# PRBonn/SHINE_mapping

Hardware: NVIDIA H100
Metric: sdf_train_points_per_sec_fwd_bwd (higher is better)
Workload: dtype f32

## Files before the change

### include/shine_b200.h

```cpp
#ifndef SHINE_B200_H_
#define SHINE_B200_H_

#include <stdint.h>

#ifdef __cplusplus
extern "C" {
#endif

#define SHINE_ABI_VERSION 5
#define SHINE_MAX_LEVELS 8
#define SHINE_HASH_SLOT_BYTES 64

#define SHINE_OK 0
#define SHINE_ERR_INVALID_ARG (-1)
#define SHINE_ERR_UNSUPPORTED (-2)
#define SHINE_ERR_CAPACITY (-3)

#define SHINE_FLAG_REDUCTION_SUM 1u
#define SHINE_FLAG_WEIGHTED 2u
#define SHINE_FLAG_TF32X1 4u
#define SHINE_FLAG_MORTON_ORDERED 16u
#define SHINE_FLAG_LOSS_L2 32u
#define SHINE_FLAG_LOSS_L1 64u

// ... 18 lines not shown

typedef struct shine_decoder {
    const float *w1, *b1, *w2, *b2, *w3, *b3;
    float *gw1, *gb1, *gw2, *gb2, *gw3, *gb3;
    int32_t in_dim;
    int32_t hidden;
    int32_t mlp_level;
    int32_t reserved;
} shine_decoder;

int shine_abi_version(void);
const char* shine_error_string(int code);

int shine_hash_insert(void* slots, uint32_t capacity, const int64_t* keys, const int32_t* corner_ids,
                      int64_t n, int32_t node_base, int32_t* overflow_count, void* stream);

int shine_points_to_morton(const float* coord, int64_t n, int32_t level, int64_t* morton, void* stream);

int shine_get_indices(const shine_octree* oct, const float* coord, int64_t n, int64_t* out_idx, void* stream);

int shine_query_fwd(const shine_octree* oct, const float* coord, int64_t n, float* out_feat, void* stream);

int shine_query_bwd(const shine_octree* oct, const float* coord, int64_t n, const float* dfeat, void* stream);

int shine_query_coord_grad(const shine_octree* oct, const float* coord, int64_t n, const float* dfeat,
                           float* out_dcoord, void* stream);
int shine_query_tangent_fwd(const shine_octree* oct, const float* coord, int64_t n, const float* tangent,
                            float* out_feat, void* stream);
int shine_query_tangent_bwd(const shine_octree* oct, const float* coord, int64_t n, const float* tangent,
                            const float* dfeat, void* stream);

int shine_sdf_infer(const shine_octree* oct, const shine_decoder* dec, const float* coord, int64_t n,
                    float* out_pred, uint8_t* out_mask, int32_t mask_level, uint32_t flags, void* stream);

int shine_sdf_fwd(const shine_octree* oct, const shine_decoder* dec, const float* coord, const float* label,
                  const float* weight, int64_t n, float sigma, float scale, float loss_scale, float* out_pred,
                  float* out_loss, uint32_t flags, void* stream);

int shine_sdf_step(const shine_octree* oct, const shine_decoder* dec, const float* coord, const float* label,
                   const float* weight, int64_t n, float sigma, float scale, float loss_scale, const float* d_loss,
                   float* out_pred, float* out_loss, uint32_t flags, void* stream);

int shine_sdf_bce_fwd(const shine_octree* oct, const shine_decoder* dec, const float* coord,
                      const float* label, const float* weight, int64_t n, float sigma, float loss_scale,
                      float* out_pred, float* out_loss, uint32_t flags, void* stream);

int shine_reduce_grad_replicas(const shine_octree* oct, void* stream);

#define SHINE_ADAM_MAX_TENSORS 16
typedef struct shine_adam_tensor {
    float* param; float* grad; float* exp_avg; float* exp_avg_sq;
    int64_t numel; float lr; float weight_decay;
} shine_adam_tensor;
int shine_adam_step(const shine_adam_tensor* tensors, int32_t count, float beta1, float beta2, float eps,
                    int32_t step, int32_t zero_grad, void* stream);

int shine_adam_step_dev(const shine_adam_tensor* tensors, int32_t count, float beta1, float beta2, float eps,
                        void* state, int32_t zero_grad, void* stream);

typedef struct shine_build_level {
    void* node_slots;
    void* corner_slots;
    void* frame_node_set;
    void* frame_corner_set;
    int32_t* node_ids_out;
    int64_t* corner_morton_out;
// ... 214 lines not shown
```

### shine_mapping_b200/_abi.py

```python
from __future__ import annotations

import ctypes as C
import os

import torch

_HERE = os.path.dirname(os.path.abspath(__file__))
LIB_PATH = os.environ.get("SHINE_B200_LIB") or os.path.join(_HERE, "csrc", "libshine_b200.so")

ABI_VERSION = 5
MAX_LEVELS = 8
HASH_SLOT_BYTES = 64
ADAM_MAX_TENSORS = 16
FLAG_REDUCTION_SUM = 1
FLAG_WEIGHTED = 2
FLAG_TF32X1 = 4
FLAG_MORTON_ORDERED = 16
FLAG_LOSS_L2 = 32
FLAG_LOSS_L1 = 64
ERR_CAPACITY = -3
REGISTER_OUT = 29
REGISTER_SCRATCH_BYTES = 1024 * REGISTER_OUT * 8
RAYCAST_MAX_REFINE = 32
CAMERA_PINHOLE = 0
# ... 76 lines not shown
class ShineCamera(C.Structure):
    _fields_ = [("model", C.c_int32), ("width", C.c_int32), ("height", C.c_int32), ("fx", C.c_float), ("fy", C.c_float),
                ("cx", C.c_float), ("cy", C.c_float), ("fov_up", C.c_float), ("fov_down", C.c_float)]


class ShineHostPool(C.Structure):
    _fields_ = [("chunks", C.c_void_p), ("chunk_shift", C.c_int32), ("num_chunks", C.c_int32), ("size", C.c_int64)]


class ShineScanInput(C.Structure):
    _fields_ = [("records", C.c_void_p), ("n", C.c_int64), ("stride_bytes", C.c_int32), ("fp64", C.c_int32)]


class ShineBrickGrid(C.Structure):
    _fields_ = [("bricks", C.c_void_p), ("sdf", C.c_void_p), ("mask", C.c_void_p), ("all_keys", C.c_void_p),
                ("num_all", C.c_int64), ("num_bricks", C.c_int64), ("origin", C.c_float * 3), ("spacing", C.c_float),
                ("n", C.c_int32), ("lo", C.c_int32 * 3), ("hi", C.c_int32 * 3), ("missing_sdf", C.c_float)]


_vp, _i64, _i32, _u32, _f32 = C.c_void_p, C.c_int64, C.c_int32, C.c_uint32, C.c_float
_OCT, _DEC = C.POINTER(ShineOctree), C.POINTER(ShineDecoder)
SYMBOLS = {
    "shine_abi_version": (C.c_int, []),
    "shine_error_string": (C.c_char_p, [C.c_int]),
    "shine_hash_insert": (C.c_int, [_vp, _u32, _vp, _vp, _i64, _i32, _vp, _vp]),
    "shine_points_to_morton": (C.c_int, [_vp, _i64, _i32, _vp, _vp]),
    "shine_get_indices": (C.c_int, [_OCT, _vp, _i64, _vp, _vp]),
    "shine_query_fwd": (C.c_int, [_OCT, _vp, _i64, _vp, _vp]),
    "shine_query_bwd": (C.c_int, [_OCT, _vp, _i64, _vp, _vp]),
    "shine_query_coord_grad": (C.c_int, [_OCT, _vp, _i64, _vp, _vp, _vp]),
    "shine_query_tangent_fwd": (C.c_int, [_OCT, _vp, _i64, _vp, _vp, _vp]),
    "shine_query_tangent_bwd": (C.c_int, [_OCT, _vp, _i64, _vp, _vp, _vp]),
    "shine_sdf_infer": (C.c_int, [_OCT, _DEC, _vp, _i64, _vp, _vp, _i32, _u32, _vp]),
    "shine_sdf_fwd": (C.c_int, [_OCT, _DEC, _vp, _vp, _vp, _i64, _f32, _f32, _f32, _vp, _vp, _u32, _vp]),
    "shine_sdf_step": (C.c_int, [_OCT, _DEC, _vp, _vp, _vp, _i64, _f32, _f32, _f32, _vp, _vp, _vp, _u32, _vp]),
    "shine_sdf_bce_fwd": (C.c_int, [_OCT, _DEC, _vp, _vp, _vp, _i64, _f32, _f32, _vp, _vp, _u32, _vp]),
    "shine_reduce_grad_replicas": (C.c_int, [_OCT, _vp]),
    "shine_octree_frame_nodes": (C.c_int, [C.POINTER(ShineBuild), _vp, _i64, _vp]),
    "shine_octree_frame_corners": (C.c_int, [C.POINTER(ShineBuild), _i32, _vp]),
    "shine_octree_sort_scratch_bytes": (C.c_int64, [_i32]),
    "shine_octree_sort_new_keys": (C.c_int, [_vp, _vp, _i32, _vp, _i64, _vp]),
    "shine_octree_assign_rows": (C.c_int, [C.POINTER(ShineBuild), _vp, _i32, _vp]),
    "shine_octree_fill_nodes": (C.c_int, [C.POINTER(ShineBuild), _vp, _i32, _vp, _vp]),
    "shine_octree_corner_rehash": (C.c_int, [_vp, _u32, _vp, _i64, _vp]),
    "shine_count_positive": (C.c_int, [_vp, _i64, _vp, _vp]),
    "shine_sdf_eikonal_step": (C.c_int, [_OCT, _DEC, _vp, _vp, _vp, _i64, _f32, _f32, _f32, _f32, _vp, _vp, _vp, _vp, _vp,
                                         _u32, _vp]),
    "shine_mark_touched": (C.c_int, [_OCT, _vp, _i64, C.POINTER(ShineTouched), _vp]),
    "shine_regularization_apply": (C.c_int, [_OCT, C.POINTER(ShineTouched), C.POINTER(ShineRowTables), _f32, _vp, _i32, _vp]),
    "shine_importance_accumulate": (C.c_int, [_OCT, C.POINTER(ShineTouched), C.POINTER(ShineRowTables), _i32, _i32, _vp]),
    "shine_boundary_pack": (C.c_int, [C.POINTER(ShineBoundary), _i32, _i32, _vp, _vp]),
    "shine_boundary_unpack": (C.c_int, [C.POINTER(ShineBoundary), _i32, _i32, _vp, _vp]),
    "shine_nccl_unique_id": (C.c_int, [_vp]),
    "shine_nccl_comm_create": (C.c_int, [_vp, _i32, _i32, _i32, C.POINTER(C.c_void_p)]),
    "shine_nccl_comm_destroy": (C.c_int, [_vp]),
    "shine_allreduce_decoder_grads": (C.c_int, [_vp, _vp, _i64, _vp]),
    "shine_comm_last_error": (C.c_char_p, []),
    "shine_p2p_create": (C.c_int, [_i32, _i32, _i32, _i64, _vp, C.POINTER(C.c_void_p)]),
    "shine_p2p_connect": (C.c_int, [_vp, _vp]),
    "shine_p2p_exchange": (C.c_int, [_vp, _vp, _i64, C.POINTER(ShineBoundary), C.POINTER(ShineBoundaryInverse), _i32, _i32, _vp]),
    "shine_p2p_timeouts": (C.c_int, [_vp, C.POINTER(C.c_int32)]),
    "shine_p2p_destroy": (C.c_int, [_vp]),
    "shine_adam_step": (C.c_int, [C.POINTER(ShineAdamTensor), _i32, _f32, _f32, _f32, _i32, _i32, _vp]),
    "shine_adam_step_dev": (C.c_int, [C.POINTER(ShineAdamTensor), _i32, _f32, _f32, _f32, _vp, _i32, _vp]),
    "shine_pool_scratch_bytes": (C.c_int64, [_i64]),
    "shine_pool_window_append": (C.c_int, [C.POINTER(ShineSamplePool), _vp, _vp, _vp, _i64, _f32, _f32, _f32, _f32, _vp,
# ... 83 lines not shown
```

### shine_mapping_b200/csrc/shine_b200.cu

```cuda

#include <cuda_runtime.h>
#include <math.h>
#include <stdint.h>

#include <type_traits>

#include "shine_b200.h"

#ifndef SHINE_GATHER_GROUP
#define SHINE_GATHER_GROUP 2
#endif
#ifndef SHINE_TRAIN_MINB
#define SHINE_TRAIN_MINB 2
#endif
#ifndef SHINE_TRAIN_DECGRAD_MINB
#define SHINE_TRAIN_DECGRAD_MINB 1
#endif
#ifndef SHINE_INFER_MINB
#define SHINE_INFER_MINB 3
#endif

#include "shine_device.cuh"

namespace {
// ... 255 lines not shown
    const float2 v = *reinterpret_cast<const float2*>(blk + 2 * c);
    split_fast2(v.x, v.y, bh.x, bh.y, bl.x, bl.y);
}
__device__ __forceinline__ void stage_afrags(float* blk, const int (&sq)[2], const float (&c)[4][4]) {
#pragma unroll
    for (int mt = 0; mt < 2; ++mt)
#pragma unroll
        for (int q = 0; q < 2; ++q)
            *reinterpret_cast<float4*>(blk + 128 * mt + 4 * sq[q]) = make_float4(c[2 * mt][q], c[2 * mt + 1][q], c[2 * mt][2 + q], c[2 * mt + 1][2 + q]);
}
__device__ __forceinline__ int xfrag_word(int ks, int c) { return 64 * ks + 2 * (c ^ (8 * ks)); }
__device__ __forceinline__ void load_xfrag(const float* sx, int ks, int c, uint2& bh, uint2& bl) {
    const float2 v = *reinterpret_cast<const float2*>(sx + xfrag_word(ks, c));
    split_fast2(v.x, v.y, bh.x, bh.y, bl.x, bl.y);
}


constexpr int kGatherGroup = SHINE_GATHER_GROUP;

using shine_internal::StepParams;

struct SmemPlan {
    static constexpr int W1 = 0;
    static constexpr int W1T = W1 + 2 * kH * kF;
    static constexpr int W2 = W1T + 2 * kF * kWS;
    static constexpr int W3W2T = W2 + 2 * kH * kWS;
    static constexpr int B1 = W3W2T + 2 * kH * kWS;
    static constexpr int B2 = B1 + kH;
    static constexpr int W3 = B2 + kH;
    static constexpr int B3 = W3 + kH;
    static constexpr int GSCALE = B3 + 1;
    static constexpr int kDecGradFloats = kH * kF + kH + kH * kH + kH + kH + 1;
    static constexpr int ZSUM = B3 + 4;
    static constexpr int H1Z = ZSUM + 8;
    static constexpr int H2Z = H1Z + kH;
    static constexpr int D2Z = H2Z + kH;
    static constexpr int DB1Z = D2Z + kH;
    static constexpr int kZsumFloats = 8 * 5 * kTile;
    static_assert(DB1Z + kH <= ZSUM + kZsumFloats, "g0 fits the zero-tile corner");
    static constexpr int STAGE = ZSUM + kZsumFloats;
    static constexpr int SB2 = 0;
    static constexpr int SU = SB2;
    static constexpr int SA1 = SB2 + kTile * kH;
    static constexpr int SX = SA1 + kTile * kH;
    static constexpr int SA2 = SX + kTile * kF;
    static constexpr int SDP = SA2;
    static constexpr int kStagePerWarp = SA2 + kTile * kH;
    static constexpr int kStageGrouped = SDP + 2 * kTile;
    __host__ __device__ static constexpr int stage_per_warp(bool grouped) { return grouped ? kStageGrouped : kStagePerWarp; }
    static constexpr int kGroupPerLevel = 4 * kTile;
    static constexpr int kW2Part = kH * kH;
};

__device__ __forceinline__ void zero_tile_gradient(float* smem, const float* __restrict__ w2, int lane) {
    const float h1 = fmaxf(smem[SmemPlan::B1 + lane], 0.f);
    float a2 = smem[SmemPlan::B2 + lane];
#pragma unroll
    for (int k = 0; k < kH; ++k) a2 = fmaf(__ldg(w2 + lane * kH + k), __shfl_sync(kFull, h1, k), a2);
    const float d2 = a2 > 0.f ? smem[SmemPlan::W3 + lane] : 0.f;
    float db1 = 0.f;
#pragma unroll
    for (int n = 0; n < kH; ++n) db1 = fmaf(__ldg(w2 + n * kH + lane), __shfl_sync(kFull, d2, n), db1);
    smem[SmemPlan::H1Z + lane] = h1;
    smem[SmemPlan::H2Z + lane] = fmaxf(a2, 0.f);
    smem[SmemPlan::D2Z + lane] = d2;
    smem[SmemPlan::DB1Z + lane] = h1 > 0.f ? db1 : 0.f;
}
__device__ __forceinline__ float zero_tile_sum_and_gradient(float* smem, const float* __restrict__ w2, int warp, int lane) {
    float s = 0.f;
#pragma unroll
    for (int w = 0; w < 8; ++w) s += smem[SmemPlan::ZSUM + w];
    if (s != 0.f) {
        if (warp == 0) zero_tile_gradient(smem, w2, lane);
        __syncthreads();
    }
    return s;
}

constexpr int kMaxGroupedRuns = 6;

__device__ __forceinline__ void red_add_f2(float* p, float a, float b) {
    asm volatile("red.global.add.v2.f32 [%0], {%1,%2};" ::"l"(p), "f"(a), "f"(b) : "memory");
}
__device__ __forceinline__ int group_slot(int p) { return 4 * (p & 3) + (p >> 2); }

template <int LMAX>
__device__ __forceinline__ void grouped_scatter(const StepParams& P, int L, int tile, const float* __restrict__ pt,
                                                float* __restrict__ dtile, const float (&dxc)[4], int lane) {
    const int g = lane >> 2, t = lane & 3;
    *reinterpret_cast<float2*>(dtile + g * kF + 2 * t) = make_float2(dxc[0], dxc[1]);
    *reinterpret_cast<float2*>(dtile + (g + 8) * kF + 2 * t) = make_float2(dxc[2], dxc[3]);
    __syncwarp();
    uint2 bh[2], bl[2];
#pragma unroll
    for (int c = 0; c < 2; ++c)
        split_fast2(dtile[(8 * c + t) * kF + g], dtile[(8 * c + t + 4) * kF + g], bh[c].x, bh[c].y, bl[c].x, bl[c].y);
    const float sx = (g & 4) ? 1.f : -1.f, ox = (g & 4) ? 0.f : 1.f;
    const float sy = (g & 2) ? 1.f : -1.f, oy = (g & 2) ? 0.f : 1.f;
    const float sz = (g & 1) ? 1.f : -1.f, oz = (g & 1) ? 0.f : 1.f;
    const int id_off = 8 * (g & 1) + 4 + (g >> 1);
    const int own = group_slot(lane & 15);
#pragma unroll
    for (int i = 0; i < LMAX; ++i) {
        if (i >= L) break;
// ... 68 lines not shown
            if (v2 >= 0) {
                const int row = __ldg(slot_words + 16 * (int64_t)v2 + id_off);
                red_add_f2(gb + (int64_t)row * kF + 2 * t, c0[2] + c1[2], c0[3] + c1[3]);
            }
        }
    }
    __syncwarp();
}

struct BatchCoords {
    __device__ __forceinline__ void load(const StepParams& P, int64_t p, float& x, float& y, float& z) const {
        x = __ldg(P.coord + 3 * p); y = __ldg(P.coord + 3 * p + 1); z = __ldg(P.coord + 3 * p + 2);
    }
    __device__ __forceinline__ float out(float v) const { return v; }
};
struct GridCoords {
    shine_internal::BrickGrid g;
    __device__ __forceinline__ void load(const StepParams&, int64_t p, float& x, float& y, float& z) const {
        const int n1 = g.n + 1, per = n1 * n1 * n1;
        const int64_t b = p / per;
        const int r = (int)(p - b * per);
        const int i = r / (n1 * n1), j = (r / n1) % n1, k = r % n1;
        x = __fadd_rn(g.origin[0], __fmul_rn(g.spacing, (float)(__ldg(g.bricks + 3 * b) * g.n + i)));
        y = __fadd_rn(g.origin[1], __fmul_rn(g.spacing, (float)(__ldg(g.bricks + 3 * b + 1) * g.n + j)));
        z = __fadd_rn(g.origin[2], __fmul_rn(g.spacing, (float)(__ldg(g.bricks + 3 * b + 2) * g.n + k)));
    }
    __device__ __forceinline__ float out(float v) const { return -v; }
};

template <class Src>
constexpr int infer_min_blocks() { return std::is_same<Src, BatchCoords>::value ? SHINE_INFER_MINB : 2; }

template <int NTF, bool TRAIN, bool DEC_GRAD, int LMAX, bool GROUPED = false, class Src = BatchCoords, int LOSS = kLossBce>
__global__ void __launch_bounds__(256, !TRAIN ? infer_min_blocks<Src>() : (DEC_GRAD && !GROUPED) ? SHINE_TRAIN_DECGRAD_MINB : SHINE_TRAIN_MINB)
sdf_fused_kernel(const __grid_constant__ StepParams P, const __grid_constant__ Src src) {
    static_assert(std::is_same<Src, BatchCoords>::value || !TRAIN, "generated coordinates are for inference only");
    static_assert(!GROUPED || TRAIN, "the grouped scatter belongs to the training kernels");
    static_assert(!DEC_GRAD || TRAIN, "decoder gradients belong to the training kernels");
    static_assert(LOSS == kLossBce || std::is_same<Src, BatchCoords>::value, "the loss belongs to labelled batches");
    static_assert(SmemPlan::kStagePerWarp >= SmemPlan::kDecGradFloats, "a warp's staging area holds its partial decoder gradient");
    static_assert(SmemPlan::kStageGrouped >= kH * kF + 3 * kH + 1, "a grouped warp's staging area holds its partial bias / dW1 gradients");
    static_assert(!(GROUPED && DEC_GRAD) ||
                      (SmemPlan::STAGE + 8 * (SmemPlan::kStageGrouped + LMAX * SmemPlan::kGroupPerLevel + SmemPlan::kW2Part)) * 4 + 1024 <=
                          227 * 1024 / SHINE_TRAIN_MINB,
                  "the grouped kernel's shared memory fits SHINE_TRAIN_MINB blocks/SM");
    extern __shared__ __align__(16) float smem[];
    uint32_t* smu = reinterpret_cast<uint32_t*>(smem);
    const int tid = threadIdx.x, lane = tid & 31, warp = tid >> 5;
    const int g = lane >> 2, t = lane & 3, odd = t & 1, half = t >> 1;
    constexpr int kWarps = 8;

    for (int i = tid; i < kH * kF; i += blockDim.x) {
        const int nrow = i / kF, k = i % kF;
        uint32_t hi, lo; split_tf32(P.dec.w1[i], hi, lo);
        smu[SmemPlan::W1 + i] = hi; smu[SmemPlan::W1 + kH * kF + i] = lo;
        smu[SmemPlan::W1T + k * kWS + nrow] = hi; smu[SmemPlan::W1T + kF * kWS + k * kWS + nrow] = lo;
    }
    for (int i = tid; i < kH * kH; i += blockDim.x) {
        const int nrow = i / kH, k = i % kH;
        const float w = P.dec.w2[i];
        uint32_t hi, lo; split_tf32(w, hi, lo);
        smu[SmemPlan::W2 + nrow * kWS + k] = hi; smu[SmemPlan::W2 + kH * kWS + nrow * kWS + k] = lo;
        split_tf32(__fmul_rn(P.dec.w3[nrow], w), hi, lo);
        smu[SmemPlan::W3W2T + k * kWS + nrow] = hi; smu[SmemPlan::W3W2T + kH * kWS + k * kWS + nrow] = lo;
    }
    if (tid < kH) {
        smem[SmemPlan::B1 + tid] = P.dec.b1 ? P.dec.b1[tid] : 0.f;
        smem[SmemPlan::B2 + tid] = P.dec.b2 ? P.dec.b2[tid] : 0.f;
        smem[SmemPlan::W3 + tid] = P.dec.w3[tid];
    }
    if (tid == 0) {
        smem[SmemPlan::B3] = P.dec.b3 ? P.dec.b3[0] : 0.f;
        smem[SmemPlan::GSCALE] = P.loss_scale * ((TRAIN && P.d_loss) ? __ldg(P.d_loss) : 1.0f);
    }
    constexpr int kPark = LMAX <= 4 ? 16 : 32;
    constexpr int kIdPark = 4 * LMAX;
    __syncthreads();
    SHINE_ACC_DECL;
#pragma unroll
    for (int a = 0; a < 2; ++a) {
#pragma unroll
        for (int b = 0; b < 4; ++b) { dW2[a][b][0] = dW2[a][b][1] = dW2[a][b][2] = dW2[a][b][3] = 0.f; }
        dW1[a][0] = dW1[a][1] = dW1[a][2] = dW1[a][3] = 0.f;
    }
#pragma unroll
    for (int j = 0; j < 4; ++j) { db2p[j][0] = db2p[j][1] = db1p[j][0] = db1p[j][1] = dw3p[j][0] = dw3p[j][1] = 0.f; }
    float dw3acc = 0.f, db2acc[4] = {0.f, 0.f, 0.f, 0.f}, db1acc[2][2] = {{0.f, 0.f}, {0.f, 0.f}};

    constexpr bool kSectorProbe = !TRAIN;
    const bool poly = P.oct.poly_interp != 0;
    const int L = P.oct.num_levels;

    float db3p = 0.f;
    float loss_acc = 0.f;

    constexpr int kStage = SmemPlan::stage_per_warp(GROUPED);
    float* stage = smem + SmemPlan::STAGE + warp * kStage;
    float* stX = stage + SmemPlan::SX;
    const int kp = g >> 2, fc = frag_chunk(lane);
    const int sq[2] = {frag_chunk(8 * t + (g & 3)), frag_chunk(8 * t + 4 + (g & 3))};
    float* gpt = smem + SmemPlan::STAGE + (DEC_GRAD ? 8 * kStage : 0) +
                 warp * (LMAX * SmemPlan::kGroupPerLevel + (DEC_GRAD ? 0 : kTile * kF));
    float* gdx = DEC_GRAD ? stX : gpt + LMAX * SmemPlan::kGroupPerLevel;
    float* w2p = smem + SmemPlan::STAGE + 8 * kStage + 8 * LMAX * SmemPlan::kGroupPerLevel + warp * SmemPlan::kW2Part;
    if (DEC_GRAD && GROUPED) {
#pragma unroll
        for (int f = 0; f < 8; ++f) *reinterpret_cast<float4*>(w2p + 128 * f + 4 * lane) = make_float4(0.f, 0.f, 0.f, 0.f);
    }

    const int warp_global = blockIdx.x * kWarps + warp;
    const int warp_stride = gridDim.x * kWarps;

    bool consecutive = true;
#pragma unroll
    for (int i = 1; i < LMAX; ++i)
        if (i < L && P.oct.lv[i].level != P.oct.lv[0].level - i) consecutive = false;

    float nx = 0.f, ny = 0.f, nz = 0.f, nlab = 0.f, nwgt = 1.f;
    bool nvalid = false;
    auto prefetch_inputs = [&](int tl) {
        const int64_t p = (int64_t)tl * kTile + g + 8 * odd;
        nvalid = tl < P.num_tiles && p < P.n;
        if (nvalid) {
            src.load(P, p, nx, ny, nz);
            if (P.label) nlab = __ldg(P.label + p);
            if (P.weighted) nwgt = fabsf(__ldg(P.weight + p));
        }
    };
    prefetch_inputs(warp_global);

    int phase = 0;
    bool advance = false;
    bool infer_exit = false;
    float pred0 = 0.f, zsum = 0.f;
    auto loss_point = [&](float pv, float lb, float wg, float& li, float& dp) {
        if constexpr (LOSS == kLossBce) {
            const float zt = __fdividef(1.0f, 1.0f + __expf(-__fdividef(lb, P.sigma)));
// ... 486 lines not shown
        }
    }

    if (P.loss && P.label) {
#pragma unroll
        for (int o = 16; o > 0; o >>= 1) loss_acc += __shfl_xor_sync(kFull, loss_acc, o);
        if (lane == 0 && loss_acc != 0.f) atomicAdd(P.loss, loss_acc * P.loss_scale);
    }
    if (DEC_GRAD) {
#pragma unroll
        for (int o = 16; o > 0; o >>= 1) zsum += __shfl_xor_sync(kFull, zsum, o);
        if (lane == 0) smem[SmemPlan::ZSUM + warp] = zsum;
    }
    if (DEC_GRAD && GROUPED) {
        float* part = stage;
        constexpr int oB1 = 256, oB2 = 288, oW3 = 320, oB3 = 352, kVec = 353;
#pragma unroll
        for (int mt = 0; mt < 2; ++mt) {
            *reinterpret_cast<float2*>(part + (16 * mt + g) * kF + 2 * t) = make_float2(dW1[mt][0], dW1[mt][1]);
            *reinterpret_cast<float2*>(part + (16 * mt + g + 8) * kF + 2 * t) = make_float2(dW1[mt][2], dW1[mt][3]);
#pragma unroll
            for (int r = 0; r < 2; ++r) {
                float d1 = db1acc[mt][r], d2 = db2acc[2 * mt + r];
#pragma unroll
                for (int o = 1; o < 4; o <<= 1) { d1 += __shfl_xor_sync(kFull, d1, o); d2 += __shfl_xor_sync(kFull, d2, o); }
                if (t == 0) { part[oB1 + 16 * mt + g + 8 * r] = d1; part[oB2 + 8 * (2 * mt + r) + g] = d2; }
            }
        }
        part[oW3 + 8 * (g >> 1) + 2 * t + (g & 1)] = dw3acc;
#pragma unroll
        for (int o = 16; o > 0; o >>= 1) db3p += __shfl_xor_sync(kFull, db3p, o);
        if (lane == 0) part[oB3] = db3p;
        __syncthreads();
        const float zs = zero_tile_sum_and_gradient(smem, P.dec.w2, warp, lane);
        for (int i = tid; i < kVec + kH * kH; i += blockDim.x) {
            float v = 0.f, g0 = 0.f;
            float* dst;
            if (i < kVec) {
#pragma unroll
                for (int w = 0; w < kWarps; ++w) v += smem[SmemPlan::STAGE + w * kStage + i];
                if (i < oB1) dst = P.dec.gw1 + i;
                else if (i < oB2) { g0 = smem[SmemPlan::DB1Z + (i - oB1)]; dst = P.dec.gb1 ? P.dec.gb1 + (i - oB1) : nullptr; }
                else if (i < oW3) {
                    v *= smem[SmemPlan::W3 + (i - oB2)]; g0 = smem[SmemPlan::D2Z + (i - oB2)];
                    dst = P.dec.gb2 ? P.dec.gb2 + (i - oB2) : nullptr;
                } else if (i < oB3) { g0 = smem[SmemPlan::H2Z + (i - oW3)]; dst = P.dec.gw3 + (i - oW3); }
                else { g0 = 1.f; dst = P.dec.gb3; }
            } else {
                const int e = i - kVec, r = e / kH, c = e % kH;
                const int f = 128 * (4 * (c >> 4) + (r >> 3)) + 4 * (4 * (c & 7) + ((r & 7) >> 1)) + 2 * ((c >> 3) & 1) + (r & 1);
#pragma unroll
                for (int w = 0; w < kWarps; ++w) v += w2p[(w - warp) * SmemPlan::kW2Part + f];
                v *= smem[SmemPlan::W3 + r];
                if (zs != 0.f) g0 = smem[SmemPlan::D2Z + r] * smem[SmemPlan::H1Z + c];
                dst = P.dec.gw2 + e;
            }
            if (zs != 0.f) v = fmaf(zs, g0, v);
            if (v != 0.f && dst) atomicAdd(dst, v);
        }
    }
    if (DEC_GRAD && !GROUPED) {
        float* part = stage;
        constexpr int oW1 = 0, oB1 = 256, oW2 = 288, oB2 = 1312, oW3 = 1344, oB3 = 1376;
        __syncwarp();
#pragma unroll
        for (int mt = 0; mt < 2; ++mt) {
#pragma unroll
            for (int nt = 0; nt < 4; ++nt) {
                *reinterpret_cast<float2*>(part + oW2 + (16 * mt + g) * kH + 8 * nt + 2 * t) = make_float2(dW2[mt][nt][0], dW2[mt][nt][1]);
                *reinterpret_cast<float2*>(part + oW2 + (16 * mt + g + 8) * kH + 8 * nt + 2 * t) = make_float2(dW2[mt][nt][2], dW2[mt][nt][3]);
            }
            *reinterpret_cast<float2*>(part + oW1 + (16 * mt + g) * kF + 2 * t) = make_float2(dW1[mt][0], dW1[mt][1]);
            *reinterpret_cast<float2*>(part + oW1 + (16 * mt + g + 8) * kF + 2 * t) = make_float2(dW1[mt][2], dW1[mt][3]);
        }
#pragma unroll
        for (int j = 0; j < 4; ++j) {
#pragma unroll
            for (int q = 0; q < 2; ++q) {
                float a = db1p[j][q], b = db2p[j][q], c = dw3p[j][q];
#pragma unroll
                for (int o = 4; o < 32; o <<= 1) {
                    a += __shfl_xor_sync(kFull, a, o); b += __shfl_xor_sync(kFull, b, o); c += __shfl_xor_sync(kFull, c, o);
                }
                if (g == 0) {
                    part[oB1 + 8 * j + 2 * t + q] = a;
                    part[oB2 + 8 * j + 2 * t + q] = b;
                    part[oW3 + 8 * j + 2 * t + q] = c;
                }
            }
        }
#pragma unroll
        for (int o = 16; o > 0; o >>= 1) db3p += __shfl_xor_sync(kFull, db3p, o);
        if (lane == 0) part[oB3] = db3p;
        __syncthreads();
        const float zs = zero_tile_sum_and_gradient(smem, P.dec.w2, warp, lane);
        for (int i = tid; i < SmemPlan::kDecGradFloats; i += blockDim.x) {
            float v = 0.f;
#pragma unroll
            for (int w = 0; w < kWarps; ++w) v += smem[SmemPlan::STAGE + w * kStage + i];
            if (zs != 0.f && i >= oB1) {
                float g0;
                if (i < oW2) g0 = smem[SmemPlan::DB1Z + (i - oB1)];
                else if (i < oB2) g0 = smem[SmemPlan::D2Z + (i - oW2) / kH] * smem[SmemPlan::H1Z + (i - oW2) % kH];
                else if (i < oW3) g0 = smem[SmemPlan::D2Z + (i - oB2)];
                else if (i < oB3) g0 = smem[SmemPlan::H2Z + (i - oW3)];
                else g0 = 1.f;
                v = fmaf(zs, g0, v);
            }
            if (v == 0.f) continue;
            float* dst;
            if (i < oB1) dst = P.dec.gw1 + i;
            else if (i < oW2) dst = P.dec.gb1 ? P.dec.gb1 + (i - oB1) : nullptr;
            else if (i < oB2) dst = P.dec.gw2 + (i - oW2);
            else if (i < oW3) dst = P.dec.gb2 ? P.dec.gb2 + (i - oB2) : nullptr;
            else if (i < oB3) dst = P.dec.gw3 + (i - oW3);
            else dst = P.dec.gb3;
            if (dst) atomicAdd(dst, v);
        }
    }
}


__global__ void __launch_bounds__(256) reduce_replicas_kernel(const __grid_constant__ shine_octree oct) {
    const shine_level& lv = oct.lv[blockIdx.y];
    if (lv.num_replicas <= 1 || !lv.grad_replicas || !lv.feature_grads) return;
    const int64_t n4 = (int64_t)lv.rows * oct.feature_dim / 4;
    float4* main4 = reinterpret_cast<float4*>(lv.feature_grads);
    float4* rep4 = reinterpret_cast<float4*>(lv.grad_replicas);
// ... 49 lines not shown
        float4 p = reinterpret_cast<float4*>(T.param)[i];
        float4 gr = reinterpret_cast<float4*>(T.grad)[i];
        float4 m = reinterpret_cast<float4*>(T.exp_avg)[i];
        float4 v = reinterpret_cast<float4*>(T.exp_avg_sq)[i];
        float* pp = &p.x; float* gg = &gr.x; float* mm = &m.x; float* vv = &v.x;
#pragma unroll
        for (int k = 0; k < 4; ++k) {
            float gk = gg[k];
            if (T.weight_decay != 0.f) gk = fmaf(T.weight_decay, pp[k], gk);
            mm[k] = mm[k] + (gk - mm[k]) * A.omb1;
            vv[k] = A.beta2 * vv[k] + A.omb2 * gk * gk;
            const float denom = sqrtf(vv[k]) / bc2_sqrt + A.eps;
            pp[k] -= step_size * (mm[k] / denom);
        }
        reinterpret_cast<float4*>(T.param)[i] = p;
        reinterpret_cast<float4*>(T.exp_avg)[i] = m;
        reinterpret_cast<float4*>(T.exp_avg_sq)[i] = v;
        if (A.zero_grad) reinterpret_cast<float4*>(T.grad)[i] = make_float4(0.f, 0.f, 0.f, 0.f);
    }
    if (blockIdx.x == 0) {
        for (int64_t i = (n4 << 2) + threadIdx.x; i < T.numel; i += blockDim.x) {
            float gk = T.grad[i];
            if (T.weight_decay != 0.f) gk = fmaf(T.weight_decay, T.param[i], gk);
            const float m = T.exp_avg[i] + (gk - T.exp_avg[i]) * A.omb1;
            const float v = A.beta2 * T.exp_avg_sq[i] + A.omb2 * gk * gk;
            T.exp_avg[i] = m; T.exp_avg_sq[i] = v;
            T.param[i] -= step_size * (m / (sqrtf(v) / bc2_sqrt + A.eps));
            if (A.zero_grad) T.grad[i] = 0.f;
        }
    }
}


template <int NTF, bool TRAIN, bool DEC_GRAD, int LMAX, bool GROUPED = false, class Src = BatchCoords, int LOSS = kLossBce>
int launch_fused_t(const StepParams& P, cudaStream_t st, const Src& src = Src()) {
    auto kern = sdf_fused_kernel<NTF, TRAIN, DEC_GRAD, LMAX, GROUPED, Src, LOSS>;
    const int smem_floats = SmemPlan::STAGE + (DEC_GRAD ? 8 * SmemPlan::stage_per_warp(GROUPED) : 0) +
                            (GROUPED ? 8 * (LMAX * SmemPlan::kGroupPerLevel + (DEC_GRAD ? SmemPlan::kW2Part : kTile * kF)) : 0);
    const size_t smem_bytes = (size_t)smem_floats * sizeof(float);
    static int per_sm_by_dev[kMaxDevices] = {0};
    int& per_sm_cached = per_sm_by_dev[current_device()];
    cudaError_t e;
    if (per_sm_cached == 0) {
        e = cudaFuncSetAttribute(kern, cudaFuncAttributeMaxDynamicSharedMemorySize, (int)smem_bytes);
        if (e != cudaSuccess) return (int)e;
        e = cudaFuncSetAttribute(kern, cudaFuncAttributePreferredSharedMemoryCarveout, cudaSharedmemCarveoutMaxShared);
        if (e != cudaSuccess) return (int)e;
        int q = 1;
        e = cudaOccupancyMaxActiveBlocksPerMultiprocessor(&q, kern, 256, smem_bytes);
        if (e != cudaSuccess) return (int)e;
        cudaFuncAttributes fa;
        e = cudaFuncGetAttributes(&fa, kern);
        if (e != cudaSuccess) return (int)e;
        const int by_regs = fa.numRegs > 0 ? 65536 / (fa.numRegs * 256) : 1;
        const int by_smem = (int)((227 * 1024) / (smem_bytes + 1024));
        int own = by_regs < by_smem ? by_regs : by_smem;
        if (own > 8) own = 8;
        if (own > q) q = own;
        per_sm_cached = q < 1 ? 1 : q;
    }
    const int per_sm = per_sm_cached;
    const int blocks_needed = (P.num_tiles + 7) / 8;
    int grid = sm_count() * per_sm;
    if (grid > blocks_needed) grid = blocks_needed;
    if (grid < 1) grid = 1;
    kern<<<grid, 256, smem_bytes, st>>>(P, src);
    return (int)cudaGetLastError();
}

template <bool TRAIN, bool DEC_GRAD, class Src = BatchCoords, int LOSS = kLossBce>
int launch_fused(const StepParams& P, uint32_t flags, cudaStream_t st, const Src& src = Src()) {
    const bool x1 = (flags & SHINE_FLAG_TF32X1) != 0;
    const bool small = P.oct.num_levels <= 4;
    if constexpr (TRAIN) {
        if ((flags & SHINE_FLAG_MORTON_ORDERED) && !x1 && small)
            return launch_fused_t<3, TRAIN, DEC_GRAD, 4, true, Src, LOSS>(P, st);
    }
    if (x1) return small ? launch_fused_t<1, TRAIN, DEC_GRAD, 4, false, Src, LOSS>(P, st, src)
                         : launch_fused_t<1, TRAIN, DEC_GRAD, 8, false, Src, LOSS>(P, st, src);
    return small ? launch_fused_t<3, TRAIN, DEC_GRAD, 4, false, Src, LOSS>(P, st, src)
                 : launch_fused_t<3, TRAIN, DEC_GRAD, 8, false, Src, LOSS>(P, st, src);
}

constexpr uint32_t kSdfFlags = SHINE_FLAG_REDUCTION_SUM | SHINE_FLAG_WEIGHTED | SHINE_FLAG_TF32X1 | SHINE_FLAG_MORTON_ORDERED;

int fill_params(StepParams& P, const shine_octree* oct, const shine_decoder* dec, const float* coord, int64_t n) {
    if (n < 0 || (n > 0 && !coord)) return SHINE_ERR_INVALID_ARG;
    if (n > (int64_t)INT32_MAX * 8) return SHINE_ERR_UNSUPPORTED;
    P.oct = *oct; P.dec = *dec; P.coord = coord; P.n = n;
    P.num_tiles = (int32_t)((n + kTile - 1) / kTile);
    P.label = nullptr; P.weight = nullptr; P.d_loss = nullptr; P.pred = nullptr; P.loss = nullptr; P.mask = nullptr;
    P.mask_level = 0; P.sigma = 1.f; P.loss_scale = 1.f; P.weighted = 0; P.scale = 1.f;
    return SHINE_OK;
}

template <bool TRAIN, bool DEC_GRAD>
int launch_loss(const StepParams& P, int loss, uint32_t flags, cudaStream_t st) {
    if (loss == kLossL1) return launch_fused<TRAIN, DEC_GRAD, BatchCoords, kLossL1>(P, flags, st);
    if (loss == kLossL2) return launch_fused<TRAIN, DEC_GRAD, BatchCoords, kLossL2>(P, flags, st);
// ... 183 lines not shown
    if (n > 0 && !out_pred) return SHINE_ERR_INVALID_ARG;
    if (out_mask && (mask_level < 0 || mask_level >= oct->num_levels)) return SHINE_ERR_INVALID_ARG;
    StepParams P;
    rc = fill_params(P, oct, dec, coord, n);
    if (rc) return rc;
    if (n == 0) return SHINE_OK;
    if ((rc = check_same_device(oct, coord))) return rc;
    DeviceGuard guard(oct->lv[0].features);
    P.pred = out_pred; P.mask = out_mask; P.mask_level = mask_level;
    return launch_fused<false, false>(P, flags, (cudaStream_t)stream);
}

int shine_sdf_fwd(const shine_octree* oct, const shine_decoder* dec, const float* coord, const float* label,
                  const float* weight, int64_t n, float sigma, float scale, float loss_scale, float* out_pred,
                  float* out_loss, uint32_t flags, void* stream) {
    return sdf_loss_call(false, oct, dec, coord, label, weight, n, sigma, scale, loss_scale, nullptr, out_pred, out_loss,
                         flags, (cudaStream_t)stream);
}

int shine_sdf_step(const shine_octree* oct, const shine_decoder* dec, const float* coord, const float* label,
                   const float* weight, int64_t n, float sigma, float scale, float loss_scale, const float* d_loss,
                   float* out_pred, float* out_loss, uint32_t flags, void* stream) {
    return sdf_loss_call(true, oct, dec, coord, label, weight, n, sigma, scale, loss_scale, d_loss, out_pred, out_loss,
                         flags, (cudaStream_t)stream);
}

int shine_sdf_bce_fwd(const shine_octree* oct, const shine_decoder* dec, const float* coord, const float* label,
                      const float* weight, int64_t n, float sigma, float loss_scale, float* out_pred, float* out_loss,
                      uint32_t flags, void* stream) {
    if (flags & (SHINE_FLAG_LOSS_L1 | SHINE_FLAG_LOSS_L2)) return SHINE_ERR_UNSUPPORTED;
    return shine_sdf_fwd(oct, dec, coord, label, weight, n, sigma, 1.f, loss_scale, out_pred, out_loss, flags, stream);
}

int shine_reduce_grad_replicas(const shine_octree* oct, void* stream) {
    int rc = check_octree(oct, false);
    if (rc) return rc;
    int64_t max_n4 = 0;
    for (int i = 0; i < oct->num_levels; ++i)
        if (oct->lv[i].num_replicas > 1 && oct->lv[i].feature_grads) {
            const int64_t n4 = (int64_t)oct->lv[i].rows * oct->feature_dim / 4;
            if (n4 > max_n4) max_n4 = n4;
        }
    if (max_n4 == 0) return SHINE_OK;
    DeviceGuard guard(oct->lv[0].features);
    int64_t blocks = (max_n4 + 255) / 256;
    const int64_t cap = (int64_t)sm_count() * 8;
    if (blocks > cap) blocks = cap;
    dim3 grid((unsigned)blocks, (unsigned)oct->num_levels);
    reduce_replicas_kernel<<<grid, 256, 0, (cudaStream_t)stream>>>(*oct);
    return (int)cudaGetLastError();
}

static int adam_check(const shine_adam_tensor* tensors, int32_t count) {
    if (!tensors || count < 1 || count > SHINE_ADAM_MAX_TENSORS) return SHINE_ERR_INVALID_ARG;
    for (int i = 0; i < count; ++i) {
        const shine_adam_tensor& t = tensors[i];
        if (!t.param || !t.grad || !t.exp_avg || !t.exp_avg_sq || t.numel < 0) return SHINE_ERR_INVALID_ARG;
        if ((((uintptr_t)t.param | (uintptr_t)t.grad | (uintptr_t)t.exp_avg | (uintptr_t)t.exp_avg_sq) & 15) != 0)
            return SHINE_ERR_INVALID_ARG;
    }
    return SHINE_OK;
}

static int adam_launch(const shine_adam_tensor* tensors, int32_t count, float beta1, float beta2, float eps, int32_t step,
                       const float* bc_dev, int32_t zero_grad, cudaStream_t st) {
    AdamParams A;
// ... 41 lines not shown
```

Before: 4.282 billion.

## Run grouped training kernel with 16 warps per block and tune smem carveout

The grouped (Morton-ordered) training kernel now launches 512 threads (16 warps) instead of 256, with shared-memory sizing, per-warp slots and the zero-tile sum generalised to the warp count. Its launch bound is relaxed to one block per SM. The launcher also sets the preferred shared-memory carveout to the fraction actually needed, falling back to max if occupancy drops, and records launch info for a new introspection API. The aim is more resident warps per block to hide gather latency, at the cost of larger per-block shared memory and tighter register limits.

New measurement: 4.369 billion, median of 6. 1.02x the previous value.

```diff
diff --git a/include/shine_b200.h b/include/shine_b200.h
--- a/include/shine_b200.h
+++ b/include/shine_b200.h
@@ -74,6 +74,8 @@
 
 int shine_sdf_infer(const shine_octree* oct, const shine_decoder* dec, const float* coord, int64_t n,
                     float* out_pred, uint8_t* out_mask, int32_t mask_level, uint32_t flags, void* stream);
+
+int shine_fused_last_launch(int32_t* out);
 
 int shine_sdf_fwd(const shine_octree* oct, const shine_decoder* dec, const float* coord, const float* label,
                   const float* weight, int64_t n, float sigma, float scale, float loss_scale, float* out_pred,
diff --git a/shine_mapping_b200/_abi.py b/shine_mapping_b200/_abi.py
--- a/shine_mapping_b200/_abi.py
+++ b/shine_mapping_b200/_abi.py
@@ -132,6 +132,7 @@
     "shine_query_tangent_fwd": (C.c_int, [_OCT, _vp, _i64, _vp, _vp, _vp]),
     "shine_query_tangent_bwd": (C.c_int, [_OCT, _vp, _i64, _vp, _vp, _vp]),
     "shine_sdf_infer": (C.c_int, [_OCT, _DEC, _vp, _i64, _vp, _vp, _i32, _u32, _vp]),
+    "shine_fused_last_launch": (C.c_int, [_vp]),
     "shine_sdf_fwd": (C.c_int, [_OCT, _DEC, _vp, _vp, _vp, _i64, _f32, _f32, _f32, _vp, _vp, _u32, _vp]),
     "shine_sdf_step": (C.c_int, [_OCT, _DEC, _vp, _vp, _vp, _i64, _f32, _f32, _f32, _vp, _vp, _vp, _u32, _vp]),
     "shine_sdf_bce_fwd": (C.c_int, [_OCT, _DEC, _vp, _vp, _vp, _i64, _f32, _f32, _vp, _vp, _u32, _vp]),
diff --git a/shine_mapping_b200/csrc/shine_b200.cu b/shine_mapping_b200/csrc/shine_b200.cu
--- a/shine_mapping_b200/csrc/shine_b200.cu
+++ b/shine_mapping_b200/csrc/shine_b200.cu
@@ -311,7 +311,7 @@
     static constexpr int GSCALE = B3 + 1;
     static constexpr int kDecGradFloats = kH * kF + kH + kH * kH + kH + kH + 1;
     static constexpr int ZSUM = B3 + 4;
-    static constexpr int H1Z = ZSUM + 8;
+    static constexpr int H1Z = ZSUM + 16;
     static constexpr int H2Z = H1Z + kH;
     static constexpr int D2Z = H2Z + kH;
     static constexpr int DB1Z = D2Z + kH;
@@ -331,6 +331,10 @@
     static constexpr int kW2Part = kH * kH;
 };
 
+__host__ __device__ constexpr int fused_warps(bool grouped) { return grouped ? 16 : 8; }
+static_assert(SmemPlan::H1Z - SmemPlan::ZSUM >= fused_warps(true) && SmemPlan::H1Z - SmemPlan::ZSUM >= fused_warps(false),
+              "every warp of a block has its zero-tile sum slot");
+
 __device__ __forceinline__ void zero_tile_gradient(float* smem, const float* __restrict__ w2, int lane) {
     const float h1 = fmaxf(smem[SmemPlan::B1 + lane], 0.f);
     float a2 = smem[SmemPlan::B2 + lane];
@@ -345,10 +349,11 @@
     smem[SmemPlan::D2Z + lane] = d2;
     smem[SmemPlan::DB1Z + lane] = h1 > 0.f ? db1 : 0.f;
 }
+template <int kWarps>
 __device__ __forceinline__ float zero_tile_sum_and_gradient(float* smem, const float* __restrict__ w2, int warp, int lane) {
     float s = 0.f;
 #pragma unroll
-    for (int w = 0; w < 8; ++w) s += smem[SmemPlan::ZSUM + w];
+    for (int w = 0; w < kWarps; ++w) s += smem[SmemPlan::ZSUM + w];
     if (s != 0.f) {
         if (warp == 0) zero_tile_gradient(smem, w2, lane);
         __syncthreads();
@@ -483,7 +488,9 @@
 constexpr int infer_min_blocks() { return std::is_same<Src, BatchCoords>::value ? SHINE_INFER_MINB : 2; }
 
 template <int NTF, bool TRAIN, bool DEC_GRAD, int LMAX, bool GROUPED = false, class Src = BatchCoords, int LOSS = kLossBce>
-__global__ void __launch_bounds__(256, !TRAIN ? infer_min_blocks<Src>() : (DEC_GRAD && !GROUPED) ? SHINE_TRAIN_DECGRAD_MINB : SHINE_TRAIN_MINB)
+__global__ void __launch_bounds__(32 * fused_warps(GROUPED),
+                                  !TRAIN ? infer_min_blocks<Src>() : GROUPED ? 1
+                                         : DEC_GRAD ? SHINE_TRAIN_DECGRAD_MINB : SHINE_TRAIN_MINB)
 sdf_fused_kernel(const __grid_constant__ StepParams P, const __grid_constant__ Src src) {
     static_assert(std::is_same<Src, BatchCoords>::value || !TRAIN, "generated coordinates are for inference only");
     static_assert(!GROUPED || TRAIN, "the grouped scatter belongs to the training kernels");
@@ -491,15 +498,15 @@
     static_assert(LOSS == kLossBce || std::is_same<Src, BatchCoords>::value, "the loss belongs to labelled batches");
     static_assert(SmemPlan::kStagePerWarp >= SmemPlan::kDecGradFloats, "a warp's staging area holds its partial decoder gradient");
     static_assert(SmemPlan::kStageGrouped >= kH * kF + 3 * kH + 1, "a grouped warp's staging area holds its partial bias / dW1 gradients");
+    constexpr int kWarps = fused_warps(GROUPED);
     static_assert(!(GROUPED && DEC_GRAD) ||
-                      (SmemPlan::STAGE + 8 * (SmemPlan::kStageGrouped + LMAX * SmemPlan::kGroupPerLevel + SmemPlan::kW2Part)) * 4 + 1024 <=
-                          227 * 1024 / SHINE_TRAIN_MINB,
-                  "the grouped kernel's shared memory fits SHINE_TRAIN_MINB blocks/SM");
+                      (SmemPlan::STAGE + kWarps * (SmemPlan::kStageGrouped + LMAX * SmemPlan::kGroupPerLevel + SmemPlan::kW2Part)) * 4 + 1024 <=
+                          227 * 1024,
+                  "the grouped kernel's shared memory fits one block per SM");
     extern __shared__ __align__(16) float smem[];
     uint32_t* smu = reinterpret_cast<uint32_t*>(smem);
     const int tid = threadIdx.x, lane = tid & 31, warp = tid >> 5;
     const int g = lane >> 2, t = lane & 3, odd = t & 1, half = t >> 1;
-    constexpr int kWarps = 8;
 
     for (int i = tid; i < kH * kF; i += blockDim.x) {
         const int nrow = i / kF, k = i % kF;
@@ -550,10 +557,10 @@
     float* stX = stage + SmemPlan::SX;
     const int kp = g >> 2, fc = frag_chunk(lane);
     const int sq[2] = {frag_chunk(8 * t + (g & 3)), frag_chunk(8 * t + 4 + (g & 3))};
-    float* gpt = smem + SmemPlan::STAGE + (DEC_GRAD ? 8 * kStage : 0) +
+    float* gpt = smem + SmemPlan::STAGE + (DEC_GRAD ? kWarps * kStage : 0) +
                  warp * (LMAX * SmemPlan::kGroupPerLevel + (DEC_GRAD ? 0 : kTile * kF));
     float* gdx = DEC_GRAD ? stX : gpt + LMAX * SmemPlan::kGroupPerLevel;
-    float* w2p = smem + SmemPlan::STAGE + 8 * kStage + 8 * LMAX * SmemPlan::kGroupPerLevel + warp * SmemPlan::kW2Part;
+    float* w2p = smem + SmemPlan::STAGE + kWarps * kStage + kWarps * LMAX * SmemPlan::kGroupPerLevel + warp * SmemPlan::kW2Part;
     if (DEC_GRAD && GROUPED) {
 #pragma unroll
         for (int f = 0; f < 8; ++f) *reinterpret_cast<float4*>(w2p + 128 * f + 4 * lane) = make_float4(0.f, 0.f, 0.f, 0.f);
@@ -1106,7 +1113,7 @@
         for (int o = 16; o > 0; o >>= 1) db3p += __shfl_xor_sync(kFull, db3p, o);
         if (lane == 0) part[oB3] = db3p;
         __syncthreads();
-        const float zs = zero_tile_sum_and_gradient(smem, P.dec.w2, warp, lane);
+        const float zs = zero_tile_sum_and_gradient<kWarps>(smem, P.dec.w2, warp, lane);
         for (int i = tid; i < kVec + kH * kH; i += blockDim.x) {
             float v = 0.f, g0 = 0.f;
             float* dst;
@@ -1167,7 +1174,7 @@
         for (int o = 16; o > 0; o >>= 1) db3p += __shfl_xor_sync(kFull, db3p, o);
         if (lane == 0) part[oB3] = db3p;
         __syncthreads();
-        const float zs = zero_tile_sum_and_gradient(smem, P.dec.w2, warp, lane);
+        const float zs = zero_tile_sum_and_gradient<kWarps>(smem, P.dec.w2, warp, lane);
         for (int i = tid; i < SmemPlan::kDecGradFloats; i += blockDim.x) {
             float v = 0.f;
 #pragma unroll
@@ -1283,11 +1290,15 @@
 }
 
 
+struct FusedLaunch { const void* kern; int per_sm, threads; size_t smem_bytes; };
+static FusedLaunch last_fused_launch[kMaxDevices] = {};
+
 template <int NTF, bool TRAIN, bool DEC_GRAD, int LMAX, bool GROUPED = false, class Src = BatchCoords, int LOSS = kLossBce>
 int launch_fused_t(const StepParams& P, cudaStream_t st, const Src& src = Src()) {
     auto kern = sdf_fused_kernel<NTF, TRAIN, DEC_GRAD, LMAX, GROUPED, Src, LOSS>;
-    const int smem_floats = SmemPlan::STAGE + (DEC_GRAD ? 8 * SmemPlan::stage_per_warp(GROUPED) : 0) +
-                            (GROUPED ? 8 * (LMAX * SmemPlan::kGroupPerLevel + (DEC_GRAD ? SmemPlan::kW2Part : kTile * kF)) : 0);
+    constexpr int kWarps = fused_warps(GROUPED), kThreads = 32 * kWarps;
+    const int smem_floats = SmemPlan::STAGE + (DEC_GRAD ? kWarps * SmemPlan::stage_per_warp(GROUPED) : 0) +
+                            (GROUPED ? kWarps * (LMAX * SmemPlan::kGroupPerLevel + (DEC_GRAD ? SmemPlan::kW2Part : kTile * kF)) : 0);
     const size_t smem_bytes = (size_t)smem_floats * sizeof(float);
     static int per_sm_by_dev[kMaxDevices] = {0};
     int& per_sm_cached = per_sm_by_dev[current_device()];
@@ -1298,24 +1309,41 @@
         e = cudaFuncSetAttribute(kern, cudaFuncAttributePreferredSharedMemoryCarveout, cudaSharedmemCarveoutMaxShared);
         if (e != cudaSuccess) return (int)e;
         int q = 1;
-        e = cudaOccupancyMaxActiveBlocksPerMultiprocessor(&q, kern, 256, smem_bytes);
+        e = cudaOccupancyMaxActiveBlocksPerMultiprocessor(&q, kern, kThreads, smem_bytes);
         if (e != cudaSuccess) return (int)e;
         cudaFuncAttributes fa;
         e = cudaFuncGetAttributes(&fa, kern);
         if (e != cudaSuccess) return (int)e;
-        const int by_regs = fa.numRegs > 0 ? 65536 / (fa.numRegs * 256) : 1;
+        const int by_regs = fa.numRegs > 0 ? 65536 / (fa.numRegs * kThreads) : 1;
         const int by_smem = (int)((227 * 1024) / (smem_bytes + 1024));
         int own = by_regs < by_smem ? by_regs : by_smem;
         if (own > 8) own = 8;
         if (own > q) q = own;
-        per_sm_cached = q < 1 ? 1 : q;
+        const int per_sm = q < 1 ? 1 : q;
+        int sm_max = 0;
+        e = cudaDeviceGetAttribute(&sm_max, cudaDevAttrMaxSharedMemoryPerMultiprocessor, current_device());
+        if (e != cudaSuccess) return (int)e;
+        const size_t need = (size_t)per_sm * (smem_bytes + 1024);
+        int pct = sm_max > 0 ? (int)((100 * need + sm_max - 1) / sm_max) : 100;
+        if (pct > 100) pct = 100;
+        e = cudaFuncSetAttribute(kern, cudaFuncAttributePreferredSharedMemoryCarveout, pct);
+        if (e != cudaSuccess) return (int)e;
+        int fit = 0;
+        e = cudaOccupancyMaxActiveBlocksPerMultiprocessor(&fit, kern, kThreads, smem_bytes);
+        if (e != cudaSuccess) return (int)e;
+        if (fit < per_sm) {
+            e = cudaFuncSetAttribute(kern, cudaFuncAttributePreferredSharedMemoryCarveout, cudaSharedmemCarveoutMaxShared);
+            if (e != cudaSuccess) return (int)e;
+        }
+        per_sm_cached = per_sm;
     }
     const int per_sm = per_sm_cached;
-    const int blocks_needed = (P.num_tiles + 7) / 8;
+    const int blocks_needed = (P.num_tiles + kWarps - 1) / kWarps;
     int grid = sm_count() * per_sm;
     if (grid > blocks_needed) grid = blocks_needed;
     if (grid < 1) grid = 1;
-    kern<<<grid, 256, smem_bytes, st>>>(P, src);
+    last_fused_launch[current_device()] = FusedLaunch{reinterpret_cast<const void*>(kern), per_sm, kThreads, smem_bytes};
+    kern<<<grid, kThreads, smem_bytes, st>>>(P, src);
     return (int)cudaGetLastError();
 }
 
@@ -1565,6 +1593,21 @@
     return shine_sdf_fwd(oct, dec, coord, label, weight, n, sigma, 1.f, loss_scale, out_pred, out_loss, flags, stream);
 }
 
+int shine_fused_last_launch(int32_t* out) {
+    if (!out) return SHINE_ERR_INVALID_ARG;
+    const FusedLaunch& L = last_fused_launch[current_device()];
+    if (!L.kern) return SHINE_ERR_INVALID_ARG;
+    cudaFuncAttributes fa;
+    cudaError_t e = cudaFuncGetAttributes(&fa, L.kern);
+    if (e != cudaSuccess) return (int)e;
+    int fit = 0;
+    e = cudaOccupancyMaxActiveBlocksPerMultiprocessor(&fit, L.kern, L.threads, L.smem_bytes);
+    if (e != cudaSuccess) return (int)e;
+    out[0] = L.per_sm; out[1] = L.threads; out[2] = (int32_t)L.smem_bytes; out[3] = fa.preferredShmemCarveout;
+    out[4] = fit; out[5] = fa.numRegs;
+    return SHINE_OK;
+}
+
 int shine_reduce_grad_replicas(const shine_octree* oct, void* stream) {
     int rc = check_octree(oct, false);
     if (rc) return rc;
```
